# arangesh/TrackMPNN

Measured on AMD Instinct MI355X. Metric: graph_edges_per_sec_fwd_bwd, higher is better.
Workload: dtype f32; 1 GPU; C2 KITTI Car/RRC-shaped rolling windows: 7 frames, D_t~clip(Poisson(6),1,20), F=8 (2d), H=64, K=0, diff; 1 fwd per frame + 1 bwd per window; 16384 windows/GPU batched block-diagonally (64 distinct seeds tiled); windows_per_gpu=16384, rows_final=6762496, parallelism=sequence-dp1

## Files before the change

trackmpnn_amd/csrc/gru_common.h:

```cpp
#pragma once
#include "common.h"
#include <algorithm>
#include <atomic>
#include <stdlib.h>

namespace tmpnn {
typedef float f32x4 __attribute__((ext_vector_type(4)));

__device__ __forceinline__ float sigmoidf_(float x) { return __builtin_amdgcn_rcpf(1.0f + __expf(-x)); }
__device__ __forceinline__ float tanhf_(float x) {
    return 1.0f - 2.0f * __builtin_amdgcn_rcpf(1.0f + __expf(2.0f * x));
}

__device__ __forceinline__ float gru_n_preact(float acc_in, float r, float hn) { return __builtin_fmaf(r, hn, acc_in); }

__device__ __forceinline__ f32x16 mfma32(float a, float b, f32x16 c) {
    return __builtin_amdgcn_mfma_f32_32x32x2f32(a, b, c, 0, 0, 0);
}

typedef __bf16 bf16x8 __attribute__((ext_vector_type(8)));
typedef __bf16 bf16x2 __attribute__((ext_vector_type(2)));

__device__ __forceinline__ uint32_t pk_bf16(float lo, float hi) {
    bf16x2 v;
    v[0] = (__bf16)lo; v[1] = (__bf16)hi;
    return __builtin_bit_cast(uint32_t, v);
}
__device__ __forceinline__ void split_pair(float x0, float x1, uint32_t& p1, uint32_t& p2, uint32_t& p3) {
    p1 = pk_bf16(x0, x1);
    float r0 = x0 - __uint_as_float(p1 << 16), r1 = x1 - __uint_as_float(p1 & 0xFFFF0000u);
    p2 = pk_bf16(r0, r1);
    r0 -= __uint_as_float(p2 << 16);
    r1 -= __uint_as_float(p2 & 0xFFFF0000u);
    p3 = pk_bf16(r0, r1);
}
struct Split8 { uint4 p1, p2, p3; };
__device__ __forceinline__ Split8 split8(const float4& u, const float4& v) {
    Split8 s;
    split_pair(u.x, u.y, s.p1.x, s.p2.x, s.p3.x);
    split_pair(u.z, u.w, s.p1.y, s.p2.y, s.p3.y);
    split_pair(v.x, v.y, s.p1.z, s.p2.z, s.p3.z);
    split_pair(v.z, v.w, s.p1.w, s.p2.w, s.p3.w);
    return s;
}
__device__ __forceinline__ f32x16 mfma_bf16(const uint4& a, const uint4& b, f32x16 c) {
    return __builtin_amdgcn_mfma_f32_32x32x16_bf16(__builtin_bit_cast(bf16x8, a), __builtin_bit_cast(bf16x8, b), c, 0, 0, 0);
}
__device__ __forceinline__ f32x16 mfma_x6(const uint4& a1, const uint4& a2, const uint4& a3, const Split8& b, f32x16 c) {
    c = mfma_bf16(a3, b.p1, c);
    c = mfma_bf16(a1, b.p3, c);
    c = mfma_bf16(a2, b.p2, c);
    c = mfma_bf16(a2, b.p1, c);
    c = mfma_bf16(a1, b.p2, c);
    c = mfma_bf16(a1, b.p1, c);
    return c;
}
__device__ __forceinline__ void split1(float x, uint16_t& q1, uint16_t& q2, uint16_t& q3) {
    uint32_t p1, p2, p3;
    split_pair(x, 0.f, p1, p2, p3);
    q1 = (uint16_t)p1; q2 = (uint16_t)p2; q3 = (uint16_t)p3;
}

__device__ __forceinline__ int acc_row(int reg, int half) { return (reg & 3) + 8 * (reg >> 2) + 4 * half; }

__device__ __forceinline__ void load16(const float* __restrict__ p, float* v) {
    const float4* q = reinterpret_cast<const float4*>(p);
#pragma unroll
    for (int i = 0; i < 4; ++i) {
        const float4 t = q[i];
        v[4 * i + 0] = t.x; v[4 * i + 1] = t.y; v[4 * i + 2] = t.z; v[4 * i + 3] = t.w;
    }
}

struct DhSrc {
    const float* d_hout; int ld_dhout;
    const float* dy; const float* w_head;
};
__device__ __forceinline__ float dh_at(const DhSrc& s, int row, int f) {
    float v = s.d_hout ? s.d_hout[(size_t)row * s.ld_dhout + f] : 0.f;
    if (s.dy) v += s.dy[row] * s.w_head[f];
    return v;
}
__device__ __forceinline__ void dh_load16(const DhSrc& s, int row, int f0, float* v) {
    if (s.d_hout) load16(s.d_hout + (size_t)row * s.ld_dhout + f0, v);
    else {
#pragma unroll
        for (int i = 0; i < 16; ++i) v[i] = 0.f;
    }
    if (s.dy) {
        const float d = s.dy[row];
        float w[16];
        load16(s.w_head + f0, w);
#pragma unroll
        for (int i = 0; i < 16; ++i) v[i] += d * w[i];
    }
}

template <int UP>
__device__ __forceinline__ float dh_at_t(const DhSrc& s, int row, int f) {
    float v = (UP & 1) ? s.d_hout[(size_t)row * s.ld_dhout + f] : 0.f;
    if (UP & 2) v += s.dy[row] * s.w_head[f];
    return v;
}
template <int UP>
__device__ __forceinline__ void dh_load16_t(const DhSrc& s, int row, int f0, float* v) {
    if (UP & 1) load16(s.d_hout + (size_t)row * s.ld_dhout + f0, v);
    else {
#pragma unroll
        for (int i = 0; i < 16; ++i) v[i] = 0.f;
    }
    if (UP & 2) {
        const float d = s.dy[row];
        float w[16];
        load16(s.w_head + f0, w);
#pragma unroll
        for (int i = 0; i < 16; ++i) v[i] += d * w[i];
    }
}

struct GruFwdArgs {
    const int32_t* rows; int R;
    const int32_t* src; const int32_t* dst;
    const float* msg; int ld_msg; int IN; int msg_compact;
    const float* h; int ld_h; int H;
    const float* wih_t; const float* whh_t; const float* b_ih; const float* b_hh;
    float* h_out; int ld_out;
    float* gates; size_t gate_plane;
    const float* w_head; float* logit_part; size_t part_stride;
};

template <int XMODE>
__device__ __forceinline__ void load_x16(const GruFwdArgs& a, int li, int row, int f0, float* v) {
    if (XMODE == 0) {
        load16(a.msg + (size_t)(a.msg_compact ? li : row) * a.ld_msg + f0, v);
    } else if (XMODE == 1) {
        float u[16], w[16];
        load16(a.h + (size_t)a.src[li] * a.ld_h + f0, u);
        load16(a.h + (size_t)a.dst[li] * a.ld_h + f0, w);
#pragma unroll
        for (int i = 0; i < 16; ++i) v[i] = u[i] - w[i];
    } else {
        if (f0 < a.H) load16(a.h + (size_t)a.src[li] * a.ld_h + f0, v);
        else          load16(a.h + (size_t)a.dst[li] * a.ld_h + (f0 - a.H), v);
    }
}


struct GruBwdDataArgs {
    const int32_t* rows; int R; int IN;
    const float* h; int ld_h; int H;
    const float* w_ih; const float* w_hh;
    const float* gates; size_t gate_plane;
    DhSrc up;
    float* d_msg; int ld_dmsg;
    float* d_h; int ld_dh;
    const int32_t* add_src; const int32_t* add_dst; const float* add_msg; int ld_add;
};

struct GruBwdWArgs {
    const int32_t* rows; int R; const int32_t* src; const int32_t* dst;
    const float* msg; int ld_msg; int IN; int msg_compact;
    const float* h; int ld_h; int H;
    const float* gates; size_t gate_plane;
    DhSrc up;
    float* slab_w;
    float* slab_b;
    int n_rs, RS, NQ, NCH;
};

template <int XMODE>
__device__ __forceinline__ float load_x1(const GruBwdWArgs& a, int lpos, int orow, int col) {
    if (XMODE == 0) return a.msg[(size_t)(a.msg_compact ? lpos : orow) * a.ld_msg + col];
    if (XMODE == 1) return a.h[(size_t)a.src[lpos] * a.ld_h + col] - a.h[(size_t)a.dst[lpos] * a.ld_h + col];
    return col < a.H ? a.h[(size_t)a.src[lpos] * a.ld_h + col] : a.h[(size_t)a.dst[lpos] * a.ld_h + col - a.H];
}

constexpr int STG_LD = 36;
template <bool NT = false, bool ACC = false>
__device__ __forceinline__ void stage_store32(float* stg, int c, int half, int lane, const f32x16& v,
                                              float* dst, int ld, int col0, int row, int r0, int R) {
#pragma unroll
    for (int q = 0; q < 4; ++q)
        *reinterpret_cast<float4*>(stg + c * STG_LD + 8 * q + 4 * half) =
            make_float4(v[4 * q], v[4 * q + 1], v[4 * q + 2], v[4 * q + 3]);
    asm volatile("s_waitcnt lgkmcnt(0)" ::: "memory");
#pragma unroll
    for (int k = 0; k < 4; ++k) {
        const int idx = k * 64 + lane;
        const int rr = idx >> 3, ch = idx & 7;
        const float4 x = *reinterpret_cast<const float4*>(stg + rr * STG_LD + ch * 4);
        const int orow = __shfl(row, rr, 64);
        if (r0 + rr < R) {
            float* p = dst + (size_t)orow * ld + col0 + ch * 4;
            if (NT) {
                __builtin_nontemporal_store(x.x, p); __builtin_nontemporal_store(x.y, p + 1);
                __builtin_nontemporal_store(x.z, p + 2); __builtin_nontemporal_store(x.w, p + 3);
            } else if (ACC) {
                const float4 o = *reinterpret_cast<const float4*>(p);
                *reinterpret_cast<float4*>(p) = make_float4(o.x + x.x, o.y + x.y, o.z + x.z, o.w + x.w);
            } else {
                *reinterpret_cast<float4*>(p) = x;
            }
        }
    }
    asm volatile("s_waitcnt lgkmcnt(0)" ::: "memory");
}

__device__ __forceinline__ void stage_rows(int row, int lane, int* orow4) {
#pragma unroll
    for (int k = 0; k < 4; ++k) orow4[k] = __shfl(row, (k * 64 + lane) >> 3, 64);
}

struct ATile { float u[16]; float w[16]; };

struct TileIdx { int li, row, s, d; };

template <int XMODE>
__device__ __forceinline__ TileIdx tile_idx(const GruFwdArgs& a, int r0, int c) {
    TileIdx t;
    t.li = min(r0 + c, a.R - 1);
    t.row = a.rows[t.li];
    t.s = (XMODE != 0) ? a.src[t.li] : 0;
    t.d = (XMODE != 0) ? a.dst[t.li] : 0;
    return t;
}


inline bool split_enabled() {
    static const int on = [] { const char* e = getenv("TMPNN_SPLIT"); return (e && e[0] == '0') ? 0 : 1; }();
    return on != 0;
}

}
```

trackmpnn_amd/csrc/gru_fwd.hip:

```cpp
#include "gru_common.h"

namespace tmpnn {

template <int CT, int XMODE>
__global__ __launch_bounds__(256, 2) void k_gru_fwd(GruFwdArgs a) {
    const int wave = threadIdx.x >> 6, lane = threadIdx.x & 63;
    const int c = lane & 31, half = lane >> 5;
    const int r0 = (blockIdx.x * 4 + wave) * 32;
    if (r0 >= a.R) return;
    const int H = a.H, H3 = 3 * a.H;
    const int col0 = blockIdx.y * (32 * CT);
    const int li = min(r0 + c, a.R - 1);
    const int row = a.rows[li];

    f32x16 acc_r[CT], acc_z[CT], acc_in[CT], acc_hn[CT];
#pragma unroll
    for (int t = 0; t < CT; ++t)
#pragma unroll
        for (int i = 0; i < 16; ++i) { acc_r[t][i] = 0.f; acc_z[t][i] = 0.f; acc_in[t][i] = 0.f; acc_hn[t][i] = 0.f; }

    for (int kt = 0; kt < a.IN / 32; ++kt) {
        const int f0 = kt * 32 + half * 16;
        float av[16];
        load_x16<XMODE>(a, li, row, f0, av);
// ... 1145 lines not shown
    }
}

template <int H, int NT>
__global__ __launch_bounds__(512) void k_rows_gemm_lds(const int32_t* __restrict__ rows, int R,
                                                       const float* __restrict__ in, int ld_in,
                                                       const float* __restrict__ wt, float* __restrict__ out,
                                                       int ld_out, int ntiles) {
    extern __shared__ float lds[];
    constexpr int NOUT = NT * 32;
    float* sW = lds;
    for (int i = threadIdx.x * 4; i < H * NOUT; i += 512 * 4)
        *reinterpret_cast<float4*>(sW + i) = *reinterpret_cast<const float4*>(wt + i);
    __syncthreads();
    const int wave = threadIdx.x >> 6, lane = threadIdx.x & 63;
    const int c = lane & 31, half = lane >> 5;
    float* stg = lds + H * NOUT + wave * (32 * STG_LD);
    for (int tile = blockIdx.x; tile < ntiles; tile += gridDim.x) {
        const int r0 = (tile * 8 + wave) * 32;
        if (r0 >= R) continue;
        const int li = min(r0 + c, R - 1);
        const int row = rows[li];
        f32x16 acc[NT];
#pragma unroll
        for (int t = 0; t < NT; ++t)
#pragma unroll
            for (int i = 0; i < 16; ++i) acc[t][i] = 0.f;
#pragma unroll
        for (int kt = 0; kt < H / 32; ++kt) {
            const int f0 = kt * 32 + half * 16;
            float av[16];
            load16(in + (size_t)row * ld_in + f0, av);
#pragma unroll
            for (int s = 0; s < 16; ++s) {
                const float* b = sW + (f0 + s) * NOUT + c;
#pragma unroll
                for (int t = 0; t < NT; ++t) acc[t] = mfma32(b[t * 32], av[s], acc[t]);
            }
        }
#pragma unroll
        for (int t = 0; t < NT; ++t) {
            stage_store32(stg, c, half, lane, acc[t], out, ld_out, t * 32, li, r0, R);
        }
    }
}

template <int H, int NT>
__global__ __launch_bounds__(512) void k_rows_gemm_split(const int32_t* __restrict__ rows, int R,
                                                         const float* __restrict__ in, int ld_in,
                                                         const float* __restrict__ wt, int ld_wt, int wt_trans,
                                                         float* __restrict__ out, int ld_out,
                                                         const int32_t* __restrict__ out_rows, int accumulate, int ntiles) {
    extern __shared__ float lds[];
    constexpr int NOUT = NT * 32, KP = H + 8, NKB = H / 16;
    uint16_t* sW = reinterpret_cast<uint16_t*>(lds);
    if (!wt_trans) {
        for (int i = threadIdx.x; i < H * NOUT / 4; i += 512) {
            const int k = i / (NOUT / 4), j0 = (i % (NOUT / 4)) * 4;
            const float4 w = *reinterpret_cast<const float4*>(wt + (size_t)k * ld_wt + j0);
            const float wv[4] = {w.x, w.y, w.z, w.w};
#pragma unroll
            for (int e = 0; e < 4; ++e) {
                uint16_t q1, q2, q3;
                split1(wv[e], q1, q2, q3);
                sW[(0 * NOUT + j0 + e) * KP + k] = q1;
                sW[(1 * NOUT + j0 + e) * KP + k] = q2;
                sW[(2 * NOUT + j0 + e) * KP + k] = q3;
            }
        }
    } else {
        for (int i = threadIdx.x; i < H * NOUT; i += 512) {
            const int n = i / H, k = i % H;
            uint16_t q1, q2, q3;
            split1(wt[(size_t)n * ld_wt + k], q1, q2, q3);
            sW[(0 * NOUT + n) * KP + k] = q1;
            sW[(1 * NOUT + n) * KP + k] = q2;
            sW[(2 * NOUT + n) * KP + k] = q3;
        }
    }
    __syncthreads();
    const int wave = threadIdx.x >> 6, lane = threadIdx.x & 63;
    const int c = lane & 31, half = lane >> 5;
    float* stg = reinterpret_cast<float*>(sW + 3 * NOUT * KP) + wave * (32 * STG_LD);
    constexpr int NQ4 = H / 8;
    float4 raw[NQ4];
    int row_n = 0, orow_n = 0;
    auto request = [&](int tile) {
        const int r0 = (tile * 8 + wave) * 32;
        if (tile < ntiles && r0 < R) {
            const int li = min(r0 + c, R - 1);
            row_n = rows ? rows[li] : li;
            orow_n = out_rows ? out_rows[li] : li;
            const float4* xr = reinterpret_cast<const float4*>(in + (size_t)row_n * ld_in + (H / 2) * half);
#pragma unroll
            for (int i = 0; i < NQ4; ++i) raw[i] = xr[i];
        }
    };
    request(blockIdx.x);
    for (int tile = blockIdx.x; tile < ntiles; tile += gridDim.x) {
        const int r0 = (tile * 8 + wave) * 32;
        if (r0 >= R) continue;
        const int orow = orow_n;
        Split8 b[NKB];
#pragma unroll
        for (int kb = 0; kb < NKB; ++kb) b[kb] = split8(raw[2 * kb], raw[2 * kb + 1]);
        request(tile + gridDim.x);
        f32x16 acc[NT];
#pragma unroll
        for (int t = 0; t < NT; ++t)
#pragma unroll
            for (int i = 0; i < 16; ++i) acc[t][i] = 0.f;
#pragma unroll
        for (int t = 0; t < NT; ++t) {
#pragma unroll
            for (int kb = 0; kb < NKB; ++kb) {
                const uint16_t* wp = sW + (t * 32 + c) * KP + (H / 2) * half + 8 * kb;
                const uint4 w1 = *reinterpret_cast<const uint4*>(wp);
                const uint4 w2 = *reinterpret_cast<const uint4*>(wp + NOUT * KP);
                const uint4 w3 = *reinterpret_cast<const uint4*>(wp + 2 * NOUT * KP);
                acc[t] = mfma_x6(w1, w2, w3, b[kb], acc[t]);
            }
        }
        if (accumulate) {
#pragma unroll
            for (int t = 0; t < NT; ++t) stage_store32<false, true>(stg, c, half, lane, acc[t], out, ld_out, t * 32, orow, r0, R);
        } else {
#pragma unroll
            for (int t = 0; t < NT; ++t) stage_store32(stg, c, half, lane, acc[t], out, ld_out, t * 32, orow, r0, R);
        }
    }
}


bool rows_gemm_supported(int KD, int NOUT) {
    if (!split_enabled() || NOUT <= 0 || NOUT % 32) return false;
    const int nt = NOUT / 32;
    return (KD == 64 && (nt == 1 || nt == 2 || nt == 4 || nt == 6)) || (KD == 32 && nt >= 1 && nt <= 3) || (KD == 128 && (nt == 1 || nt == 2));
}
int launch_rows_gemm(const int32_t* rows, int R, const float* in, int ld_in, int KD, const float* wt, int ld_wt, int wt_trans,
                     int NOUT, float* out, int ld_out, const int32_t* out_rows, int accumulate, hipStream_t st) {
    if (R <= 0) return TMPNN_OK;
    if (!rows_gemm_supported(KD, NOUT)) return set_error(TMPNN_EINVAL, "rows_gemm: unsupported shape KD=%d NOUT=%d", KD, NOUT);
    TM_REQUIRE(in && wt && out && ld_in >= KD && (ld_in & 3) == 0 && aligned16(in) && (ld_out & 3) == 0 && aligned16(out) &&
                   (wt_trans || ((ld_wt & 3) == 0 && aligned16(wt))), "rows_gemm: rows must be 16-byte aligned");
    const int ntiles = ceil_div(R, 256);
    dim3 grid(ntiles < 256 ? ntiles : 256), block(512);
    const size_t shm2 = (size_t)3 * NOUT * (KD + 8) * 2 + sizeof(float) * 8 * 32 * STG_LD;
#define RG(HH, NN)                                                                                                  \
    do {                                                                                                            \
        TM_SHM_ONCE((k_rows_gemm_split<HH, NN>), shm2);                                                             \
        hipLaunchKernelGGL((k_rows_gemm_split<HH, NN>), grid, block, shm2, st, rows, R, in, ld_in, wt, ld_wt, wt_trans, out, \
                           ld_out, out_rows, accumulate, ntiles);                                                   \
    } while (0)
    const int nt = NOUT / 32;
    if (KD == 128)     { if (nt == 1) RG(128, 1); else RG(128, 2); }
    else if (KD == 64) { if (nt == 1) RG(64, 1); else if (nt == 2) RG(64, 2); else if (nt == 4) RG(64, 4); else RG(64, 6); }
    else               { if (nt == 1) RG(32, 1); else if (nt == 2) RG(32, 2); else RG(32, 3); }
#undef RG
    return check_launch("rows_gemm_split");
}

}

using namespace tmpnn;

extern "C" {


int tmpnn_gru_fwd_head_parts(int H, int IN, int xmode) {
    if (H != 32 && H != 64) return 0;
    const size_t wpb = (H == 64) ? 12 : 8;
    const size_t shm = sizeof(float) * ((size_t)((xmode == 3 ? 0 : IN) + H) * 3 * H + wpb * 32 * STG_LD + 4);
    return shm > 160 * 1024 ? 0 : H / 32;
}

int tmpnn_gru_fwd(const int32_t* rows, int R, int xmode, const int32_t* src, const int32_t* dst, const float* msg,
                  int ld_msg, int msg_compact, int IN, const float* h, int ld_h, int H, const float* wih_t, const float* whh_t,
                  const float* b_ih, const float* b_hh, float* h_out, int ld_out, float* gates, size_t gate_plane,
                  const float* w_head, float* logit_part, size_t part_stride, tmpnn_stream stream) {
    TM_REQUIRE(supported_H_cell(H), "gru_fwd: unsupported H=%d", H);
    TM_REQUIRE(R >= 0, "gru_fwd: R=%d", R);
    if (R == 0) return TMPNN_OK;
    TM_REQUIRE(xmode >= 0 && xmode <= 3, "gru_fwd: xmode=%d", xmode);
    TM_REQUIRE(IN == (xmode == 2 ? 2 * H : (xmode == 1 || xmode == 3 ? H : IN)) && IN % 32 == 0 && IN > 0,
               "gru_fwd: IN=%d does not match xmode=%d H=%d", IN, xmode, H);
    TM_REQUIRE(rows && h && whh_t && b_ih && b_hh && h_out && (wih_t || xmode == 3), "gru_fwd: null pointer");
    TM_REQUIRE(xmode == 0 ? (msg != nullptr && ld_msg >= IN && (ld_msg & 3) == 0 && aligned16(msg))
                          : (src != nullptr && dst != nullptr),
               "gru_fwd: message source missing/misaligned for xmode=%d", xmode);
    TM_REQUIRE(xmode != 3 || (H <= 64 && msg != nullptr && ld_msg >= 3 * H && (ld_msg & 3) == 0 && aligned16(msg)),
               "gru_fwd: xmode 3 needs H <= 64 and the projected det rows msg [Dn][3H]");
    TM_REQUIRE(ld_h >= H && ld_out >= H && (ld_h & 3) == 0 && aligned16(h), "gru_fwd: bad state layout");
    TM_REQUIRE(gates == nullptr || gate_plane >= (size_t)H, "gru_fwd: gate_plane too small");
    TM_REQUIRE(logit_part == nullptr || (w_head != nullptr && aligned16(w_head) && tmpnn_gru_fwd_head_parts(H, IN, xmode) > 0),
               "gru_fwd: fused head not available for H=%d IN=%d xmode=%d (see tmpnn_gru_fwd_head_parts)", H, IN, xmode);
    GruFwdArgs a{rows, R, src, dst, msg, ld_msg, IN, msg_compact, h, ld_h, H, wih_t, whh_t, b_ih, b_hh, h_out, ld_out, gates,
                 gate_plane, w_head, logit_part, part_stride};
    hipStream_t st = as_stream(stream);
    if (H <= 64 && (xmode == 3 || aligned16(wih_t)) && aligned16(whh_t) && aligned16(h_out) && (ld_out & 3) == 0 && aligned16(b_ih) &&
        aligned16(b_hh) && (gates == nullptr || (aligned16(gates) && (gate_plane & 3) == 0))) {
        const int rows_per_pass = (H == 64) ? 192 : 256;
        const int ntiles = ceil_div(R, rows_per_pass);
        dim3 pgrid(ntiles < 256 ? ntiles : 256), pblock(H == 64 ? 768 : 512);
        const int wpb = (H == 64) ? 12 : 8;
        if (xmode == 3 && split_enabled()) {
            const size_t shm2 = (size_t)3 * 3 * H * (H + 8) * 2 + sizeof(float) * ((size_t)8 * 32 * STG_LD + 4 + 5 * H);
            if (H == 64) {
                TM_SHM_ONCE((k_gru_fwd_split<64, 8>), shm2);
                hipLaunchKernelGGL((k_gru_fwd_split<64, 8>), pgrid, dim3(512), shm2, st, a);
            } else {
                TM_SHM_ONCE((k_gru_fwd_split<32, 8>), shm2);
                hipLaunchKernelGGL((k_gru_fwd_split<32, 8>), pgrid, dim3(512), shm2, st, a);
            }
            return check_launch("gru_fwd_split");
        }
        if (xmode == 0 && IN == H && split_enabled() && aligned16(msg) && aligned16(wih_t)) {
            const size_t shmn = (size_t)2 * 3 * 96 * (H + 8) * 2 + sizeof(float) * ((size_t)8 * 32 * STG_LD + 4 + 5 * 32);
            const int cwn = H / 32;
            const int want = ceil_div(ceil_div(R, 32), 8);
            int groups = want < 256 / cwn ? want : 256 / cwn;
            groups = (groups + 7) & ~7;
            dim3 ngrid(groups * cwn);
            if (H == 64) {
                TM_SHM_ONCE((k_gru_fwd_split_node<64, 8>), shmn);
                hipLaunchKernelGGL((k_gru_fwd_split_node<64, 8>), ngrid, dim3(512), shmn, st, a);
            } else {
                TM_SHM_ONCE((k_gru_fwd_split_node<32, 8>), shmn);
                hipLaunchKernelGGL((k_gru_fwd_split_node<32, 8>), ngrid, dim3(512), shmn, st, a);
            }
            return check_launch("gru_fwd_split_node");
        }
        const size_t shm = sizeof(float) * ((size_t)((xmode == 3 ? 0 : IN) + H) * 3 * H + (size_t)wpb * 32 * STG_LD + 4);
        if (shm > 160 * 1024) goto generic;
#define LL(HH, II, X, CC, WW)                                                                                \
    do {                                                                                                     \
        TM_SHM_ONCE((k_gru_fwd_lds<HH, II, X, CC, WW>), shm);                     \
        hipLaunchKernelGGL((k_gru_fwd_lds<HH, II, X, CC, WW>), pgrid, pblock, shm, st, a, ntiles);           \
    } while (0)
        if (H == 64) { if (xmode == 0 && IN == 64) LL(64, 64, 0, 1, 12); else if (xmode == 1) LL(64, 64, 1, 1, 12); else if (xmode == 2) LL(64, 128, 2, 1, 12); else if (xmode == 3) LL(64, 64, 3, 1, 12); else goto generic; }
        else         { if (xmode == 0 && IN == 32) LL(32, 32, 0, 1, 8); else if (xmode == 1) LL(32, 32, 1, 1, 8); else if (xmode == 2) LL(32, 64, 2, 1, 8); else if (xmode == 3) LL(32, 32, 3, 1, 8); else goto generic; }
#undef LL
        return check_launch("gru_fwd_lds");
    }
generic:
    TM_REQUIRE(logit_part == nullptr, "gru_fwd: fused head requested but the LDS path is unavailable (alignment)");
    TM_REQUIRE(xmode != 3, "gru_fwd: xmode 3 is only available on the LDS path (H <= 64, 16-byte aligned buffers)");
    int CT = (H % 64 == 0) ? 2 : 1;
    if (CT == 2 && (long)ceil_div(R, 128) * (H / 64) < 128) CT = 1;
    dim3 grid(ceil_div(R, 128), H / (32 * CT)), block(256);
#define L(C, X) hipLaunchKernelGGL((k_gru_fwd<C, X>), grid, block, 0, st, a)
    if (CT == 2) { if (xmode == 0) L(2, 0); else if (xmode == 1) L(2, 1); else L(2, 2); }
    else         { if (xmode == 0) L(1, 0); else if (xmode == 1) L(1, 1); else L(1, 2); }
#undef L
    return check_launch("gru_fwd");
}

int tmpnn_gru_fwd_tiles(const tmpnn_edge_tiles* tiles, int R, const float* proj, int ld_proj, const float* h, int ld_h, int H,
                        const float* whh_t, const float* b_ih, const float* b_hh, float* h_out, int ld_out, float* gates,
                        size_t gate_plane, const float* w_head, float* logit_part, size_t part_stride, tmpnn_stream stream) {
    TM_REQUIRE(H == 32 || H == 64, "gru_fwd_tiles: H=%d (the tiled forward serves the LDS-resident cells, H in {32, 64})", H);
    TM_REQUIRE(R >= 0, "gru_fwd_tiles: R=%d", R);
    if (R == 0) return TMPNN_OK;
    TM_REQUIRE(split_enabled(), "gru_fwd_tiles: the tiled forward is the bf16x6 form (TMPNN_SPLIT=0 keeps tmpnn_gru_fwd)");
    TM_REQUIRE(tiles != nullptr, "gru_fwd_tiles: tiles is null");
    const int RPT = tiles->rows_per_tile;
    TM_REQUIRE((RPT == 32 || RPT == 16) && tiles->T > 0 && (long)tiles->T * RPT >= R && (long)(tiles->T - 1) * RPT < R &&
                   tiles->t_row && tiles->t_loc && tiles->t_dptr && tiles->t_dets,
               "gru_fwd_tiles: tile list (T=%d, rows_per_tile=%d) does not cover R=%d rows in 16- or 32-row tiles", tiles->T,
               tiles->rows_per_tile, R);
    TM_REQUIRE(proj && h && whh_t && b_ih && b_hh && h_out, "gru_fwd_tiles: null pointer");
    TM_REQUIRE(ld_proj >= 3 * H && (ld_proj & 3) == 0 && aligned16(proj) && ld_h >= H && ld_out >= H && (ld_h & 3) == 0 &&
                   aligned16(h) && aligned16(whh_t) && aligned16(h_out) && (ld_out & 3) == 0 && aligned16(b_ih) && aligned16(b_hh) &&
                   (gates == nullptr || (aligned16(gates) && (gate_plane & 3) == 0 && gate_plane >= (size_t)H)),
               "gru_fwd_tiles: layout (16-byte alignment, leading dimensions)");
    TM_REQUIRE(logit_part == nullptr || (w_head != nullptr && aligned16(w_head)), "gru_fwd_tiles: fused head needs a 16-byte aligned w_head");
    GruFwdArgs a{nullptr, R, nullptr, nullptr, proj, ld_proj, H, 0, h, ld_h, H, nullptr, whh_t, b_ih, b_hh, h_out, ld_out, gates,
                 gate_plane, w_head, logit_part, part_stride};
    FwdTiles tl{tiles->t_row, tiles->t_loc, tiles->t_dptr, tiles->t_dets, tiles->T};
    hipStream_t st = as_stream(stream);
    const int ntiles = ceil_div(R, (H == 64) ? 192 : 256);
    dim3 pgrid(ntiles < 256 ? ntiles : 256);
    if (RPT == 16) {
        const size_t shm16 = (size_t)3 * 3 * H * H * 2 + sizeof(float) * ((size_t)16 * T16_AREA + 4 + 5 * H);
        if (H == 64) {
            TM_SHM_ONCE((k_gru_fwd_split_t16<64, 16>), shm16);
            hipLaunchKernelGGL((k_gru_fwd_split_t16<64, 16>), pgrid, dim3(1024), shm16, st, a, tl);
        } else {
            TM_SHM_ONCE((k_gru_fwd_split_t16<32, 16>), shm16);
            hipLaunchKernelGGL((k_gru_fwd_split_t16<32, 16>), pgrid, dim3(1024), shm16, st, a, tl);
        }
        return check_launch("gru_fwd_split_t16");
    }
    const size_t shm = (size_t)3 * 3 * H * (H + 8) * 2 + sizeof(float) * ((size_t)8 * TP_AREA + 4 + 5 * H);
    if (H == 64) {
        TM_SHM_ONCE((k_gru_fwd_split_tiled<64, 8>), shm);
        hipLaunchKernelGGL((k_gru_fwd_split_tiled<64, 8>), pgrid, dim3(512), shm, st, a, tl);
    } else {
        TM_SHM_ONCE((k_gru_fwd_split_tiled<32, 8>), shm);
        hipLaunchKernelGGL((k_gru_fwd_split_tiled<32, 8>), pgrid, dim3(512), shm, st, a, tl);
    }
    return check_launch("gru_fwd_split_tiled");
}

int tmpnn_gru_fwd_tiles_zero_state_available(int H, int xmode) { return (H == 32 || H == 64) && xmode == 3 && split_enabled(); }

int tmpnn_gru_fwd_tiles_zero_state(const tmpnn_edge_tiles* tiles, int R, const float* proj, int ld_proj, int H,
                                   const float* b_ih, const float* b_hh, float* h_out, int ld_out, float* gates,
                                   size_t gate_plane, int write_hn, const float* w_head, float* logit_part, size_t part_stride,
                                   tmpnn_stream stream) {
    TM_REQUIRE(tmpnn_gru_fwd_tiles_zero_state_available(H, 3), "gru_fwd_tiles_zero_state: H=%d (H in {32, 64}, TMPNN_SPLIT on)", H);
    TM_REQUIRE(R >= 0, "gru_fwd_tiles_zero_state: R=%d", R);
    if (R == 0) return TMPNN_OK;
    TM_REQUIRE(tiles != nullptr, "gru_fwd_tiles_zero_state: tiles is null");
    TM_REQUIRE(tiles->rows_per_tile == 32 && tiles->T > 0 && (long)tiles->T * 32 >= R && (long)(tiles->T - 1) * 32 < R &&
                   tiles->t_row && tiles->t_loc && tiles->t_dptr && tiles->t_dets,
               "gru_fwd_tiles_zero_state: tile list (T=%d, rows_per_tile=%d) does not cover R=%d rows in 32-row tiles", tiles->T,
               tiles->rows_per_tile, R);
    TM_REQUIRE(proj && b_ih && b_hh && h_out, "gru_fwd_tiles_zero_state: null pointer");
    TM_REQUIRE(ld_proj >= 3 * H && (ld_proj & 3) == 0 && aligned16(proj) && ld_out >= H && aligned16(h_out) && (ld_out & 3) == 0 &&
                   aligned16(b_ih) && aligned16(b_hh) &&
                   (gates == nullptr || (aligned16(gates) && (gate_plane & 3) == 0 && gate_plane >= (size_t)H)),
               "gru_fwd_tiles_zero_state: layout (16-byte alignment, leading dimensions)");
    TM_REQUIRE(logit_part == nullptr || (w_head != nullptr && aligned16(w_head)),
               "gru_fwd_tiles_zero_state: fused head needs a 16-byte aligned w_head");
    GruFwdArgs a{nullptr, R, nullptr, nullptr, proj, ld_proj, H, 0, nullptr, 0, H, nullptr, nullptr, b_ih, b_hh, h_out, ld_out,
                 gates, gate_plane, w_head, logit_part, part_stride};
    FwdTiles tl{tiles->t_row, tiles->t_loc, tiles->t_dptr, tiles->t_dets, tiles->T, write_hn ? 1 : 0};
    hipStream_t st = as_stream(stream);
    const int ntiles = ceil_div(R, (H == 64) ? 96 : 128);
    dim3 pgrid(ntiles < 768 ? ntiles : 768);
    const size_t shm = sizeof(float) * ((size_t)4 * TP_AREA + 4 + 5 * H);
    if (H == 64) {
        TM_SHM_ONCE((k_gru_fwd_split_tiled<64, 4, true>), shm);
        hipLaunchKernelGGL((k_gru_fwd_split_tiled<64, 4, true>), pgrid, dim3(256), shm, st, a, tl);
    } else {
        TM_SHM_ONCE((k_gru_fwd_split_tiled<32, 4, true>), shm);
        hipLaunchKernelGGL((k_gru_fwd_split_tiled<32, 4, true>), pgrid, dim3(256), shm, st, a, tl);
    }
    return check_launch("gru_fwd_split_tiled_zs");
}

int tmpnn_rows_linear(const int32_t* rows, int R, const float* in, int ld_in, int H, const float* wt, int NOUT,
                      float* out, int ld_out, tmpnn_stream stream) {
    TM_REQUIRE((H == 32 || H == 64) && (NOUT == 3 * H), "rows_linear: only [H<=64] x [3H] projections (H=%d NOUT=%d)", H, NOUT);
    if (R == 0) return TMPNN_OK;
    TM_REQUIRE(R > 0 && rows && in && wt && out, "rows_linear: null pointer");
    TM_REQUIRE(ld_in >= H && (ld_in & 3) == 0 && aligned16(in) && aligned16(wt) && ld_out >= NOUT && (ld_out & 3) == 0 &&
                   aligned16(out),
               "rows_linear: rows must be 16-byte aligned");
    const int ntiles = ceil_div(R, 256);
    dim3 grid(ntiles < 256 ? ntiles : 256), block(512);
    hipStream_t st = as_stream(stream);
    if (split_enabled()) return launch_rows_gemm(rows, R, in, ld_in, H, wt, NOUT, 0, NOUT, out, ld_out, nullptr, 0, st);
    const size_t shm = sizeof(float) * ((size_t)H * NOUT + 8 * 32 * STG_LD);
    if (H == 64) {
        TM_SHM_ONCE((k_rows_gemm_lds<64, 6>), shm);
        hipLaunchKernelGGL((k_rows_gemm_lds<64, 6>), grid, block, shm, st, rows, R, in, ld_in, wt, out, ld_out, ntiles);
    } else {
        TM_SHM_ONCE((k_rows_gemm_lds<32, 3>), shm);
        hipLaunchKernelGGL((k_rows_gemm_lds<32, 3>), grid, block, shm, st, rows, R, in, ld_in, wt, out, ld_out, ntiles);
    }
    return check_launch("rows_linear");
}

}
```

Measured before the change: 746.3 million graph-edges/s.

## Add row-streaming zero-state GRU forward kernel with software-pipelined gathers

Adds a dedicated kernel for the zero-state H=64 GRU forward with no gates output. Each 16-lane group walks a contiguous chunk of rows and computes the gates elementwise from gathered projections, instead of using the tiled MFMA kernel with shared-memory staging. Index loads and projection gathers are software-pipelined one row ahead, and the source row is reused while the source detection stays the same. The fused head logit is reduced with DPP row shifts. This targets the latency of the gather-bound tiled path and its shared-memory overhead, at the cost of relying on sequential row order for load reuse.

```diff
diff --git a/trackmpnn_amd/csrc/gru_common.h b/trackmpnn_amd/csrc/gru_common.h
--- a/trackmpnn_amd/csrc/gru_common.h
+++ b/trackmpnn_amd/csrc/gru_common.h
@@ -226,6 +226,10 @@
 }
 
 
+int launch_gru_fwd_zs_rows(const int32_t* t_row, const int32_t* t_loc, const int32_t* t_dptr, const int32_t* t_dets, int R,
+                           const float* proj, int ld_proj, const float* b_ih, const float* b_hh, float* h_out, int ld_out,
+                           const float* w_head, float* logit_part, size_t part_stride, hipStream_t st);
+
 inline bool split_enabled() {
     static const int on = [] { const char* e = getenv("TMPNN_SPLIT"); return (e && e[0] == '0') ? 0 : 1; }();
     return on != 0;
diff --git a/trackmpnn_amd/csrc/gru_fwd.hip b/trackmpnn_amd/csrc/gru_fwd.hip
--- a/trackmpnn_amd/csrc/gru_fwd.hip
+++ b/trackmpnn_amd/csrc/gru_fwd.hip
@@ -1471,6 +1471,15 @@
     return check_launch("gru_fwd_split_tiled");
 }
 
+static bool zs_rows_enabled() {
+#ifdef TMPNN_KEEP_VARIANTS
+    static const bool v = [] { const char* e = getenv("TMPNN_ZS_FWD_ROWS"); return e == nullptr || e[0] != '0'; }();
+    return v;
+#else
+    return true;
+#endif
+}
+
 int tmpnn_gru_fwd_tiles_zero_state_available(int H, int xmode) { return (H == 32 || H == 64) && xmode == 3 && split_enabled(); }
 
 int tmpnn_gru_fwd_tiles_zero_state(const tmpnn_edge_tiles* tiles, int R, const float* proj, int ld_proj, int H,
@@ -1496,6 +1505,9 @@
                  gates, gate_plane, w_head, logit_part, part_stride};
     FwdTiles tl{tiles->t_row, tiles->t_loc, tiles->t_dptr, tiles->t_dets, tiles->T, write_hn ? 1 : 0};
     hipStream_t st = as_stream(stream);
+    if (H == 64 && gates == nullptr && zs_rows_enabled())
+        return launch_gru_fwd_zs_rows(tiles->t_row, tiles->t_loc, tiles->t_dptr, tiles->t_dets, R, proj, ld_proj, b_ih, b_hh,
+                                      h_out, ld_out, w_head, logit_part, part_stride, st);
     const int ntiles = ceil_div(R, (H == 64) ? 96 : 128);
     dim3 pgrid(ntiles < 768 ? ntiles : 768);
     const size_t shm = sizeof(float) * ((size_t)4 * TP_AREA + 4 + 5 * H);
diff --git a/trackmpnn_amd/csrc/gru_fwd_zs_rows.hip b/trackmpnn_amd/csrc/gru_fwd_zs_rows.hip
--- /dev/null
+++ b/trackmpnn_amd/csrc/gru_fwd_zs_rows.hip
@@ -0,0 +1,137 @@
+#include "gru_common.h"
+
+namespace tmpnn {
+
+struct ZsRowsArgs {
+    const int32_t* t_row; const int32_t* t_loc; const int32_t* t_dptr; const int32_t* t_dets;
+    const float* proj; int ld_proj;
+    const float* b_ih; const float* b_hh;
+    float* h_out; int ld_out;
+    const float* w_head; float* logit_part; size_t part_stride;
+    int R, chunk;
+};
+
+__device__ __forceinline__ float zsr_gate(float ps, float pd, float bsum) { return sigmoidf_((0.0f + (ps - pd)) + bsum); }
+__device__ __forceinline__ float zsr_gate_n(float ps, float pd, float b_in, float r, float hn) {
+    return tanhf_(gru_n_preact((ps - pd) + b_in, r, hn));
+}
+__device__ __forceinline__ float zsr_out(float z, float n) { return (1.0f - z) * n + z * 0.0f; }
+
+template <int N>
+__device__ __forceinline__ float row_up(float v) {
+    return __builtin_bit_cast(float, __builtin_amdgcn_update_dpp(0, __builtin_bit_cast(int, v), 0x100 + N, 0xF, 0xF, true));
+}
+
+__device__ __forceinline__ float4 ld4(const float* p) { return *reinterpret_cast<const float4*>(p); }
+
+struct ZsPass {
+    int loc, dp;
+    int sdet, ddet;
+    int row, held;
+    float4 s0, s1, s2, d0, d1, d2;
+};
+
+struct ZsConst { float b_r[4], b_z[4], b_in[4], hn[4], w[4]; };
+
+struct ZsOut { float4 o; float part; int row; bool live; };
+
+__device__ __forceinline__ void zs_rows_store(const ZsRowsArgs& a, bool head, int j, const ZsOut& r) {
+    if (!r.live) return;
+    *reinterpret_cast<float4*>(a.h_out + (size_t)r.row * a.ld_out + 4 * j) = r.o;
+    if (head && (j & 7) == 0) a.logit_part[(size_t)(j >> 3) * a.part_stride + r.row] = r.part;
+}
+
+__device__ __forceinline__ void zs_rows_pass(const ZsRowsArgs& a, const ZsConst& k, int p, int hi, bool warm, bool head, int j,
+                                             const ZsPass& cu, ZsPass& nx, ZsOut& res) {
+    constexpr int H = 64;
+    const int c0 = 4 * j, last = a.R - 1;
+    zs_rows_store(a, head, j, res);
+    res.live = false;
+    const int qa = min(p + 3, last);
+    nx.loc = a.t_loc[qa];
+    nx.dp = a.t_dptr[qa >> 5];
+    nx.sdet = a.t_dets[cu.dp + (cu.loc & 0xFFFF)];
+    nx.ddet = a.t_dets[cu.dp + (int)((unsigned)cu.loc >> 16)];
+    nx.row = a.t_row[min(max(p + 1, 0), last)];
+    const float* pd = a.proj + (size_t)cu.ddet * a.ld_proj + c0;
+    nx.d0 = ld4(pd); nx.d1 = ld4(pd + H); nx.d2 = ld4(pd + 2 * H);
+    nx.s0 = cu.s0; nx.s1 = cu.s1; nx.s2 = cu.s2;
+    nx.held = cu.sdet;
+    if (cu.sdet != cu.held) {
+        const float* ps = a.proj + (size_t)cu.sdet * a.ld_proj + c0;
+        nx.s0 = ld4(ps); nx.s1 = ld4(ps + H); nx.s2 = ld4(ps + 2 * H);
+    }
+    if (warm) return;
+    const float sr[4] = {cu.s0.x, cu.s0.y, cu.s0.z, cu.s0.w}, dr[4] = {cu.d0.x, cu.d0.y, cu.d0.z, cu.d0.w};
+    const float sz[4] = {cu.s1.x, cu.s1.y, cu.s1.z, cu.s1.w}, dz[4] = {cu.d1.x, cu.d1.y, cu.d1.z, cu.d1.w};
+    const float sn[4] = {cu.s2.x, cu.s2.y, cu.s2.z, cu.s2.w}, dn[4] = {cu.d2.x, cu.d2.y, cu.d2.z, cu.d2.w};
+    float o[4];
+#pragma unroll
+    for (int e = 0; e < 4; ++e) {
+        const float ro = zsr_gate(sr[e], dr[e], k.b_r[e]);
+        const float zo = zsr_gate(sz[e], dz[e], k.b_z[e]);
+        const float no = zsr_gate_n(sn[e], dn[e], k.b_in[e], ro, k.hn[e]);
+        o[e] = zsr_out(zo, no);
+    }
+    res.o = make_float4(o[0], o[1], o[2], o[3]);
+    res.row = cu.row;
+    res.live = p < hi && cu.row >= 0;
+    if (head) {
+        const float g = o[0] * k.w[0] + o[1] * k.w[1] + o[2] * k.w[2] + o[3] * k.w[3];
+        float ph = 0.f;
+        ph += g;
+        ph += row_up<2>(g);
+        ph += row_up<4>(g);
+        ph += row_up<6>(g);
+        ph += row_up<1>(ph);
+        res.part = ph;
+    }
+}
+
+__global__ __launch_bounds__(256, 5) void k_gru_fwd_zs_rows(ZsRowsArgs a) {
+    constexpr int H = 64;
+    const int lane = threadIdx.x & 63, j = lane & 15, c0 = 4 * j;
+    const int grp = (blockIdx.x * 4 + (threadIdx.x >> 6)) * 4 + (lane >> 4);
+    const bool head = a.logit_part != nullptr;
+
+    ZsConst k;
+    {
+        const float4 ir = ld4(a.b_ih + c0), hr = ld4(a.b_hh + c0);
+        const float4 iz = ld4(a.b_ih + H + c0), hz = ld4(a.b_hh + H + c0);
+        const float4 in = ld4(a.b_ih + 2 * H + c0), hh = ld4(a.b_hh + 2 * H + c0);
+        k.b_r[0] = ir.x + hr.x; k.b_r[1] = ir.y + hr.y; k.b_r[2] = ir.z + hr.z; k.b_r[3] = ir.w + hr.w;
+        k.b_z[0] = iz.x + hz.x; k.b_z[1] = iz.y + hz.y; k.b_z[2] = iz.z + hz.z; k.b_z[3] = iz.w + hz.w;
+        k.b_in[0] = in.x; k.b_in[1] = in.y; k.b_in[2] = in.z; k.b_in[3] = in.w;
+        k.hn[0] = 0.0f + hh.x; k.hn[1] = 0.0f + hh.y; k.hn[2] = 0.0f + hh.z; k.hn[3] = 0.0f + hh.w;
+        const float4 wh = head ? ld4(a.w_head + c0) : make_float4(0.f, 0.f, 0.f, 0.f);
+        k.w[0] = wh.x; k.w[1] = wh.y; k.w[2] = wh.z; k.w[3] = wh.w;
+    }
+
+    const long lo_l = (long)grp * a.chunk;
+    const int lo = (int)(lo_l < a.R ? lo_l : a.R);
+    const int hi = min(a.R, lo + a.chunk);
+
+    const float4 z4 = make_float4(0.f, 0.f, 0.f, 0.f);
+    ZsPass x{0, 0, 0, 0, -1, -1, z4, z4, z4, z4, z4, z4}, y = x;
+    ZsOut res{z4, 0.f, -1, false};
+#pragma unroll 1
+    for (int i = -3; i < a.chunk; i += 2) {
+        zs_rows_pass(a, k, lo + i, hi, i < 0, head, j, x, y, res);
+        zs_rows_pass(a, k, lo + i + 1, hi, i + 1 < 0, head, j, y, x, res);
+    }
+    zs_rows_store(a, head, j, res);
+}
+
+int launch_gru_fwd_zs_rows(const int32_t* t_row, const int32_t* t_loc, const int32_t* t_dptr, const int32_t* t_dets, int R,
+                           const float* proj, int ld_proj, const float* b_ih, const float* b_hh, float* h_out, int ld_out,
+                           const float* w_head, float* logit_part, size_t part_stride, hipStream_t st) {
+    constexpr int GROUPS_PER_BLOCK = 16, MIN_CHUNK = 8, MAX_BLOCKS = 2048;
+    const int want = ceil_div(R, GROUPS_PER_BLOCK * MIN_CHUNK);
+    const int blocks = want < MAX_BLOCKS ? want : MAX_BLOCKS;
+    const int chunk = ceil_div(R, (long)blocks * GROUPS_PER_BLOCK);
+    ZsRowsArgs a{t_row, t_loc, t_dptr, t_dets, proj, ld_proj, b_ih, b_hh, h_out, ld_out, w_head, logit_part, part_stride, R, chunk};
+    hipLaunchKernelGGL(k_gru_fwd_zs_rows, dim3(blocks), dim3(256), 0, st, a);
+    return check_launch("gru_fwd_zs_rows");
+}
+
+}
```

After: 736.1 million graph-edges/s. -1.4%, worse.
